# EternityJune25/ComoRAG

Hardware: AMD Instinct MI355X
Metric: top-k queries/sec (higher is better)
Workload: dtype bf16; 1 GPU; brute-force top-20 over 10000000 x 768 bf16 rows, batch 64, row-sharded over 1 GPU(s) (north_star target config); rows=10000000, dim=768, batch=64, k=20, query_batches_rotated=4, device=AMD Radeon Graphics (gfx950:sramecc+:xnack-), n_cu=256, repeats=1, exchange=none (1 shard)

## Files before the change

comorag_amd/csrc/api.hip:

```cpp
#include <hip/hip_runtime.h>

#include <algorithm>
#include <cmath>
#include <cstdarg>
#include <cstdio>
#include <cstdlib>
#include <cstring>
#include <chrono>
#include <atomic>
#include <climits>
#include <map>
#include <memory>
#include <mutex>
#include <shared_mutex>
#include <string>
#include <vector>

#include "../../include/comorag_hip.h"
#include "cmr_kernels.h"
#include "cmr_internal.h"
#include "index_state.h"
#include "search_plan.h"
#include "prefilter_host.h"

// ... 10 lines not shown
    g_err = buf;
    return code;
}
#define fail cmr_fail

int cmr_set_device(int device) {
    HIP_TRY(hipSetDevice(device));
    return CMR_OK;
}

namespace {

struct Option {
    const char* name;
    void (*store)(cmr_index*, long long);
    enum Kind { any, clamp, oneof, range, zero_or } kind;
    long long a, b, c;
    const char* reject;
    long long (*read)(const cmr_index*);
};
#define CMR_STR_(x) #x
#define CMR_STR(x) CMR_STR_(x)
#define OPT_FIELD(f) [](cmr_index* i, long long v) { i->f = (decltype(i->f))v; }
#define OPT_READ(expr) [](const cmr_index* i) -> long long { return expr; }
const Option kOptions[] = {
    {"scan_ring", OPT_FIELD(force_ring), Option::any, 0, 0, 0, nullptr, nullptr},
    {"scan_asm_ring", OPT_FIELD(force_asm), Option::any, 0, 0, 0, nullptr, nullptr},
    {"scan_grid", OPT_FIELD(force_grid), Option::any, 0, 0, 0, nullptr, nullptr},
    {"scan_no_sample", OPT_FIELD(no_sample), Option::any, 0, 0, 0, nullptr, nullptr},
    {"scan_no_wide", OPT_FIELD(no_wide), Option::any, 0, 0, 0, nullptr, nullptr},
    {"scan_no_tiny", OPT_FIELD(no_tiny), Option::any, 0, 0, 0, nullptr, nullptr},
    {"scan_no_small", OPT_FIELD(no_small), Option::any, 0, 0, 0, nullptr, nullptr},
    {"small_max_panels", OPT_FIELD(small_max_panels), Option::clamp, 32, 6144, 0, nullptr, nullptr},
    {"tiny_multi", OPT_FIELD(tiny_multi), Option::any, 0, 0, 0, nullptr, nullptr},
    {"zero_copy", OPT_FIELD(zero_copy), Option::any, 0, 0, 0, nullptr, nullptr},
    {"sample_single", OPT_FIELD(single_level), Option::any, 0, 0, 0, nullptr, nullptr},
    {"sample_single_max", OPT_FIELD(single_level_max), Option::clamp, 0, LLONG_MAX, 0, nullptr, nullptr},
    {"sample_tau_in_scan", OPT_FIELD(tau_in_scan), Option::any, 0, 0, 0, nullptr, nullptr},
    {"scan_fin", OPT_FIELD(scan_fin), Option::any, 0, 0, 0, nullptr, nullptr},
    {"sync_poll", OPT_FIELD(sync_poll), Option::any, 0, 0, 0, nullptr, nullptr},
    {"scan_fin_dense", OPT_FIELD(fin_dense), Option::clamp, 1, 1 << 16, 0, nullptr, nullptr},
    {"scan_fin_cap", OPT_FIELD(fin_cap), Option::oneof, 0, 128, 256, "scan_fin_cap must be 0, 128 or 256", nullptr},
    {"scan_fin_suppliers", OPT_FIELD(fin_suppliers), Option::clamp, 0, CMR_FIN_SLOTS / CMR_SCAN_WAVES, 0, nullptr, nullptr},
    {"scan_fin_spin", OPT_FIELD(fin_spin), Option::clamp, 0, 1000, 0, nullptr, nullptr},
    {"scan_fin_queries", OPT_FIELD(fin_max_q), Option::clamp, 1, CMR_FIN_MAX_QUERIES, 0, nullptr, nullptr},
    {"sample_div", OPT_FIELD(sample_div), Option::clamp, 2, LLONG_MAX, 0, nullptr, nullptr},
    {"sample_maxmul", OPT_FIELD(sample_maxmul), Option::clamp, 0, LLONG_MAX, 0, nullptr, nullptr},
    {"pipe_reserve_cus", OPT_FIELD(reserve_cus), Option::any, 0, 0, 0, nullptr, nullptr},
    {"pipe_slots", OPT_FIELD(pipe_slots), Option::any, 0, 0, 0, nullptr, nullptr},
    {"wide_mode", OPT_FIELD(wide_mode), Option::range, 0, 2, 0, "wide_mode must be 0 (default), 1 (register-resident kernel) or 2 (query-split grid)", nullptr},
    {"stream_nt", OPT_FIELD(stream_nt), Option::any, 0, 0, 0, nullptr, nullptr},
    {"pipe_dual_scan", OPT_FIELD(dual_scan), Option::any, 0, 0, 0, nullptr, nullptr},
    {"pipe_cu_mask", OPT_FIELD(cu_mask), Option::any, 0, 0, 0, nullptr, nullptr},
    {"exact_cand", OPT_FIELD(exact_cand), Option::range, 2, CMR_MAX_K, 0, "exact_cand must be in [2, " CMR_STR(CMR_MAX_K) "]", OPT_READ(i->exact_cand)},
    {"combine", [](cmr_index* i, long long v) { i->combine.store((int)v, std::memory_order_relaxed); }, Option::zero_or, 2, cmr_combine::kMaxWidth, 0,
     "combine must be 0 (off) or in [2, " CMR_STR(CMR_PPR_MAX_BATCH) "]", OPT_READ(i->combine.load(std::memory_order_relaxed))},
    {"combine_wait_us", [](cmr_index* i, long long v) { i->combine_wait_us.store(v, std::memory_order_relaxed); }, Option::clamp, 0, 10000000, 0, nullptr,
     OPT_READ(i->combine_wait_us.load(std::memory_order_relaxed))},
    {"combine_filtered", [](cmr_index* i, long long v) { i->combine_filtered.store((int)v, std::memory_order_relaxed); }, Option::range, 0, 1, 0,
     "combine_filtered must be 0 or 1", OPT_READ(i->combine_filtered.load(std::memory_order_relaxed))},
    {"prefilter", OPT_FIELD(prefilter), Option::range, -1, 2, 0, "prefilter must be -1 (auto), 0 (off), 1 (on) or 2 (on, the filter keeps every row)", OPT_READ(i->prefilter)},
    {"prefilter_rescore_wgs", OPT_FIELD(pf_rescore_wgs), Option::clamp, 0, 1024, 0, nullptr, nullptr},
    {"prefilter_tighten", OPT_FIELD(pf_tighten), Option::range, 0, 1, 0, "prefilter_tighten must be 0 or 1", OPT_READ(i->pf_tighten)},
    {"prefilter_pair_cap", OPT_FIELD(pf_pair_cap), Option::clamp, 0, 1 << 20, 0, nullptr, OPT_READ(i->pf_pair_cap)},
    {"prefilter_wave_cap", OPT_FIELD(pf_wave_cap), Option::clamp, 0, 1 << 20, 0, nullptr, OPT_READ(i->pf_wave_cap)},
    {"prefilter_sample", OPT_FIELD(pf_sample), Option::range, -1, 1, 0, "prefilter_sample must be -1 (auto), 0 (bf16 sampling) or 1 (int8 sample)", OPT_READ(i->pf_sample)},
    {"prefilter_sample_panels", OPT_FIELD(pf_sample_panels), Option::clamp, 0, INT_MAX, 0, nullptr, OPT_READ(i->pf_sample_panels)},
    {"prefilter_sample_run", OPT_FIELD(pf_sample_run), Option::clamp, 0, 1 << 16, 0, nullptr, OPT_READ(i->pf_sample_run)},
    {"prefilter_sample_wave_cap", OPT_FIELD(pf_sample_wave_cap), Option::clamp, 0, 1 << 20, 0, nullptr, OPT_READ(i->pf_sample_wave_cap)},
    {"prefilter_sample_level0", OPT_FIELD(pf_sample_level0), Option::clamp, 0, 128, 0, nullptr, OPT_READ(i->pf_sample_level0)},
    {"prefilter_sample_active", nullptr, Option::any, 0, 0, 0, nullptr, OPT_READ(i->prefilter_sample_active)},
    {"prefilter_sample_pairs", nullptr, Option::any, 0, 0, 0, nullptr, OPT_READ(q8_read_counter(i, Q8Counter::sample_pairs))},
    {"prefilter_sample_overflow", nullptr, Option::any, 0, 0, 0, nullptr, OPT_READ(q8_read_counter(i, Q8Counter::sample_overflow))},
    {"prefilter_active", nullptr, Option::any, 0, 0, 0, nullptr, OPT_READ(i->prefilter_active)},
    {"prefilter_rows", nullptr, Option::any, 0, 0, 0, nullptr, OPT_READ(i->q8c.q8 ? i->q8c.rows : 0)},
    {"prefilter_bytes", nullptr, Option::any, 0, 0, 0, nullptr, OPT_READ((long long)i->q8c.bytes(i->dpad))},
    {"prefilter_candidates", nullptr, Option::any, 0, 0, 0, nullptr, OPT_READ(q8_read_counter(i, Q8Counter::candidates))},
    {"prefilter_pairs", nullptr, Option::any, 0, 0, 0, nullptr, OPT_READ(q8_read_counter(i, Q8Counter::pairs))},
    {"prefilter_pair_overflow", nullptr, Option::any, 0, 0, 0, nullptr, OPT_READ(q8_read_counter(i, Q8Counter::pair_overflow))},
    {"prefilter_wave_overflow", nullptr, Option::any, 0, 0, 0, nullptr, OPT_READ(q8_read_counter(i, Q8Counter::wave_overflow))},
    {"last_route", nullptr, Option::any, 0, 0, 0, nullptr, OPT_READ(i->last_route.load(std::memory_order_relaxed))},
    {"pipe_dual_scan_active", nullptr, Option::any, 0, 0, 0, nullptr, OPT_READ(i->dual_active)},
    {"pipe_dual_scan_wide_active", nullptr, Option::any, 0, 0, 0, nullptr, OPT_READ(i->dual_wide_active)},
    {"pipe_cu_mask_active", nullptr, Option::any, 0, 0, 0, nullptr, OPT_READ(i->pipe.last_masked)},
    {"pipe_scan_cus", nullptr, Option::any, 0, 0, 0, nullptr, OPT_READ(i->pipe.last_masked ? i->pipe.scan_cus : i->n_cu)},
    {"combine_batches", nullptr, Option::any, 0, 0, 0, nullptr, OPT_READ(i->combiner.batches())},
    {"combine_queries", nullptr, Option::any, 0, 0, 0, nullptr, OPT_READ(i->combiner.queries())},
    {"combine_max_width", nullptr, Option::any, 0, 0, 0, nullptr, OPT_READ(i->combiner.max_width())},
};
#undef OPT_FIELD
#undef OPT_READ

const Option* find_option(const char* name) {
    for (const Option& o : kOptions) if (strcmp(o.name, name) == 0) return &o;
    return nullptr;
}

int set_option(cmr_index* idx, const char* name, long long v) {
    const Option* o = find_option(name ? name : "");
    if (!o || !o->store) return fail(CMR_ERR_INVALID, "unknown option '%s'", name ? name : "");
    const bool refused = o->kind == Option::oneof ? (v != o->a && v != o->b && v != o->c) : o->kind == Option::range ? (v < o->a || v > o->b) : o->kind == Option::zero_or ? (v != 0 && (v < o->a || v > o->b)) : false;
    if (refused) return fail(CMR_ERR_INVALID, "%s", o->reject);
    if (o->kind == Option::clamp) v = std::max(o->a, std::min(v, o->b));
    o->store(idx, v);
    return CMR_OK;
}
// ... 181 lines not shown
    {
        std::lock_guard<std::mutex> pg(idx->prof_mu);
        prof = idx->prof_on && (idx->prof_seq++ % (unsigned)idx->prof_every) == 0;
    }
    if (prof) {
        HIP_TRY(hipEventCreate(&pe.a));
        HIP_TRY(hipEventCreate(&pe.b));
        HIP_TRY(hipEventRecord(pe.a, sm));
    }
    const int* fin_state = nullptr;
    if (p.fin) {
        if (!ws->fin_ctl_armed) {
            HIP_TRY(ws->fin_ctl.ensure(p.bytes.fin_ctl));
            HIP_TRY(hipMemsetAsync(ws->fin_ctl.p, 0, p.bytes.fin_ctl, sm));
            ws->fin_ctl_armed = true;
        }
        HIP_TRY(ws->fin_pmax.ensure(p.bytes.fin_pmax));
        HIP_TRY(ws->fin_tau.ensure(p.bytes.fin_tau));
        HIP_TRY(ws->fin_mm.ensure(p.bytes.fin_mm));
        a.fin_mm = (u64*)ws->fin_mm.p;
        HIP_TRY(ws->fin_dense.ensure(p.bytes.fin_dense));
        a.fin = (int*)ws->fin_ctl.p; a.fin_pmax = (u64*)ws->fin_pmax.p; a.fin_tau = (u64*)ws->fin_tau.p; a.fin_dense = (u64*)ws->fin_dense.p;
        a.fin_first = p.fin_first; a.fin_wgs = p.fin_wgs; a.fin_mul = p.fin_mul; a.fin_dcap = p.fin_dcap; a.fin_spin = p.fin_spin;
        a.out_ids = ids_dev; a.out_scores = scores_dev; a.out_min = min_dev; a.out_max = max_dev; a.id_base = kernel_id_base(idx);
        fin_state = (const int*)ws->fin_ctl.p + CMR_FIN_STATE;
        if (ws->done_ptr && idx->single_block()) a.fin_done = ws->done_ptr;
    }
    if (p.prefilter) { if ((rc = q8_filter(idx, f, a, sm))) return rc; }
    else HIP_TRY(p.wide ? cmr_launch_scan_wide(g, a, sm) : p.fin ? cmr_launch_scan_fin(g, a, sm) : p.masked_each ? cmr_launch_scan_masked_each(g, a, sm) : p.masked ? cmr_launch_scan_masked(g, a, sm) : cmr_launch_scan_topk(g, a, sm));
    if (prof) {
        HIP_TRY(hipEventRecord(pe.b, sm));
        std::lock_guard<std::mutex> pg(idx->prof_mu);
        idx->prof_events.push_back(pe);
        idx->prof_bytes = p.prefilter ? prefilter_bytes(idx, p) : algorithmic_bytes(idx, nqp, k);
    }
    if (a.fin_done) {
        ws->lazy.due = true;
        ws->lazy.lists = (const u64*)ws->lists.p; ws->lazy.cnt = (const int*)ws->cnt.p; ws->lazy.W = p.W; ws->lazy.NQ = p.NQ; ws->lazy.cap = g.cap; ws->lazy.nqp = nqp; ws->lazy.k = k;
        ws->lazy.mm = (const float2*)ws->mm.p; ws->lazy.id_base = kernel_id_base(idx); ws->lazy.ids = ids_dev; ws->lazy.scores = scores_dev; ws->lazy.mn = min_dev; ws->lazy.mx = max_dev;
        ws->lazy.state = fin_state;
        ws->done_used = true;
        return CMR_OK;
    }
    if (sq != sm) {
        HIP_TRY(hipEventRecord(st.ev_scan, sm));
        HIP_TRY(hipStreamWaitEvent(sq, st.ev_scan, 0));
    }
    if (p.prefilter && (rc = q8_rescore(f, sq))) return rc;
    HIP_TRY(cmr_launch_merge_query((const u64*)ws->lists.p, (const int*)ws->cnt.p, p.W, p.NQ, g.cap, nqp, k, (const float2*)ws->mm.p,
                                   kernel_id_base(idx), ids_dev, scores_dev, min_dev, max_dev, nullptr, sq, G > 1, fin_state));
    return remap_ids_enqueue(idx, ids_dev, (long long)nqp * k, sq);
}

int plan_and_enqueue_pass(cmr_index* idx, Workspace* ws, const PassStreams& st, const PassSplit& ps, int k, int reserve_cus, const float* q_dev,
                          const float* min_score, int64_t* ids_dev, float* scores_dev, float* min_dev, float* max_dev, int prefilter = 0) {
    PassPlan plan;
    PassRequest rq = st.request(ps.nqp, k, ps.route, min_score != nullptr, reserve_cus);
    rq.prefilter = prefilter;
    int rc = plan_pass(idx, rq, &plan);
    if (rc) return rc;
    if (ps.q0 == 0)
        idx->last_route.store(route_code(plan, min_score != nullptr) | (ps.nqp < ps.nq ? CMR_ROUTE_MORE_PASSES : 0), std::memory_order_relaxed);
    return enqueue_pass(idx, ws, st, plan, q_dev + (size_t)ps.q0 * idx->dim, min_score, ids_dev + (size_t)ps.q0 * k, scores_dev + (size_t)ps.q0 * k,
                        min_dev ? min_dev + ps.q0 : nullptr, max_dev ? max_dev + ps.q0 : nullptr);
}

int search_enqueue(cmr_index* idx, Workspace* ws, const float* q_dev, int nq, int k, int64_t* ids_dev, float* scores_dev,
                   float* min_dev, float* max_dev, const float* min_score = nullptr) {
    if (k > CMR_MAX_K) {
        if (min_score) return fail(CMR_ERR_UNSUPPORTED, "threshold search supports k <= %d", CMR_MAX_K);
        return search_large_k_enqueue(idx, ws, q_dev, nq, k, ids_dev, scores_dev, min_dev, max_dev);
    }
    if (const int kind = small_path_kind(idx, nq, k, min_score != nullptr)) {
        const long long npanels = idx->npanels();
        idx->last_route.store(route_code(kind == 1 ? CMR_ROUTE_TINY : CMR_ROUTE_SMALL), std::memory_order_relaxed);
        { int rc_ = arm_flag(ws, ws->stream); if (rc_) return rc_; }
        HIP_TRY(ws->d_out.ensure(cmr_tiny_scratch_bytes(nq, (int)npanels, k, idx->tiny_multi, idx->small_max_panels)));
        if (!ws->arrive.p) {
            HIP_TRY(ws->arrive.ensure(sizeof(int)));
            HIP_TRY(hipMemsetAsync(ws->arrive.p, 0, sizeof(int), ws->stream));
        }
        HIP_TRY(cmr_launch_tiny_search(idx->dtype, idx->corpus, q_dev, nq, idx->dim, idx->dpad, idx->n, k, kernel_id_base(idx), ws->d_out.p,
                                       ids_dev, scores_dev, min_dev, max_dev, ws->flag_ptr, idx->tiny_multi ? (int*)ws->arrive.p : nullptr, idx->small_max_panels, ws->stream,
                                       (ws->done_ptr && idx->single_block()) ? ws->done_ptr : nullptr));
        if (ws->done_ptr && idx->single_block()) ws->done_used = true;
        return remap_ids_enqueue(idx, ids_dev, (long long)nq * k, ws->stream);
    }
    const PassStreams st = PassStreams::one(ws->stream);
    for (PassSplit ps(idx, nq); ps.next();) {
        int rc = plan_and_enqueue_pass(idx, ws, st, ps, k, 0, q_dev, min_score, ids_dev, scores_dev, min_dev, max_dev);
        if (rc) return rc;
    }
    return CMR_OK;
}

int search_masked_enqueue(cmr_index* idx, Workspace* ws, const float* q_dev, int nq, int k, const unsigned* allow_dev, int64_t* ids_dev,
                          float* scores_dev, float* min_dev, float* max_dev, long long mask_stride = 0) {
    const PassStreams st = PassStreams::one(ws->stream);
    const int per_pass = idx->narrow_width(nq);
    for (int q0 = 0; q0 < nq; q0 += per_pass) {
        const int nqp = std::min(per_pass, nq - q0);
        PassPlan plan;
        PassRequest rq = st.request(nqp, k, Route::narrow, false, 0);
        rq.masked = true;
        rq.masked_each = mask_stride > 0;
        int rc = plan_pass(idx, rq, &plan);
        if (rc) return rc;
        if (q0 == 0) idx->last_route.store(route_code(plan, false) | (nqp < nq ? CMR_ROUTE_MORE_PASSES : 0), std::memory_order_relaxed);
        rc = enqueue_pass(idx, ws, st, plan, q_dev + (size_t)q0 * idx->dim, nullptr, ids_dev + (size_t)q0 * k, scores_dev + (size_t)q0 * k,
                          min_dev ? min_dev + q0 : nullptr, max_dev ? max_dev + q0 : nullptr, allow_dev + (size_t)q0 * (size_t)mask_stride, mask_stride);
        if (rc) return rc;
    }
    return CMR_OK;
}

int create_pipe_streams(cmr_index* idx, Pipe& T, int mask, bool dual) {
    HIP_TRY(hipStreamCreateWithFlags(&T.st[Pipe::sq], hipStreamNonBlocking));
// ... 10 lines not shown
        uint32_t scan[8], rest[8];
        for (int w = 0; w < 8; ++w) {
            scan[w] = mask == 2 ? 0x00FFFFFFu : (w < 6 ? 0xFFFFFFFFu : 0u);
            rest[w] = ~scan[w];
        }
        HIP_TRY(hipExtStreamCreateWithCUMask(&T.st[Pipe::sm], 8, scan));
        if (dual) HIP_TRY(hipExtStreamCreateWithCUMask(&T.st[Pipe::sm2], 8, scan));
        HIP_TRY(hipExtStreamCreateWithCUMask(&T.st[Pipe::sp], 8, rest));
        T.scan_cus = idx->n_cu - 64;
        for (Pipe::Stream u : {Pipe::usp, Pipe::usm, Pipe::uwp, Pipe::uwm}) HIP_TRY(hipStreamCreateWithFlags(&T.st[u], hipStreamNonBlocking));
    } else {
        HIP_TRY(hipStreamCreateWithFlags(&T.st[Pipe::wp], hipStreamNonBlocking));
        HIP_TRY(hipStreamCreateWithFlags(&T.st[Pipe::wm], hipStreamNonBlocking));
        HIP_TRY(hipStreamCreateWithFlags(&T.st[Pipe::sp], hipStreamNonBlocking));
        HIP_TRY(hipStreamCreateWithFlags(&T.st[Pipe::sm], hipStreamNonBlocking));
        if (dual) HIP_TRY(hipStreamCreateWithFlags(&T.st[Pipe::sm2], hipStreamNonBlocking));
    }
    return CMR_OK;
}
int ensure_pipe(cmr_index* idx) {
    Pipe& P = idx->pipe;
    if (P.st[Pipe::sq]) return CMR_OK;
    int mask = idx->cu_mask < 0 ? (idx->n_cu == 256 ? 1 : 0) : (idx->n_cu == 256 ? idx->cu_mask : 0);
    hipEvent_t ev[CMR_PIPE_SLOTS][3] = {};
    Pipe T;
    auto undo = [&]() {
        T.destroy_streams();
        for (auto& slot : ev) for (hipEvent_t& e : slot) if (e) { (void)hipEventDestroy(e); e = nullptr; }
        T.scan_cus = T.wide_cus = 0;
    };
    int rc = create_pipe_streams(idx, T, mask, idx->dual_scan < 0 ? mask != 0 : idx->dual_scan != 0);
    if (rc && mask) {
        undo();
        mask = 0;
        rc = create_pipe_streams(idx, T, 0, idx->dual_scan > 0);
    }
    if (rc) { undo(); return rc; }
    auto make_events = [&]() -> int {
        for (auto& slot : ev) for (hipEvent_t& e : slot) HIP_TRY(hipEventCreateWithFlags(&e, hipEventDisableTiming));
        return CMR_OK;
    };
    rc = make_events();
    if (rc) { undo(); return rc; }
    for (int i = 0; i < Pipe::n_streams; ++i) if (i != Pipe::sq) P.st[i] = T.st[i];
    P.scan_cus = T.scan_cus; P.wide_cus = T.wide_cus;
    for (int i = 0; i < CMR_PIPE_SLOTS; ++i) {
        P.slot[i].pre_done = ev[i][0]; P.slot[i].main_done = ev[i][1]; P.slot[i].scan_done = ev[i][2];
        P.slot[i].ws.stream = P.st[Pipe::sm];
    }
    P.st[Pipe::sq] = T.st[Pipe::sq];
    return CMR_OK;
}

int search_pipelined_enqueue_locked(cmr_index* idx, const float* q_dev, int nq, int k, int64_t* ids_dev, float* scores_dev, float* min_dev,
                                    float* max_dev, hipEvent_t wait_event, hipEvent_t* done_event, const float* min_score, bool may_prefilter = false) {
    Pipe& P = idx->pipe;
    { int rc_ = ensure_pipe(idx); if (rc_) return rc_; }
    P.nslots = std::min(CMR_PIPE_SLOTS, std::max(2, idx->pipe_slots));
    if (k > CMR_MAX_K) return fail(CMR_ERR_UNSUPPORTED, "pipelined search supports k <= %d", CMR_MAX_K);
    const bool masked = P.scan_cus != 0 && (idx->cu_mask > 0 || idx->short_scan());
    const bool twins = P.scan_cus != 0 && !masked;
    P.last_masked = masked ? 1 : 0;
    hipStream_t const nsp = P.st[twins ? Pipe::usp : Pipe::sp], wsp = P.st[twins ? Pipe::uwp : Pipe::wp];
    PassSplit ps(idx, nq);
    if (wait_event) {
        HIP_TRY(hipStreamWaitEvent(nsp, wait_event, 0));
        if (ps.any_wide()) HIP_TRY(hipStreamWaitEvent(wsp, wait_event, 0));
    }
    int prefilter = prefilter_eligible(idx, min_score != nullptr, min_dev || max_dev, nq, may_prefilter);
    if (prefilter && !q8_ensure_companion(idx, nsp)) prefilter = 0;
    idx->prefilter_active = 0;
    idx->prefilter_sample_active = 0;
    PipeSlot* last = nullptr;
    while (ps.next()) {
        const bool wide = ps.wide_streams();
        PipeSlot* sl = &P.slot[P.next++ % (unsigned)P.nslots];
        hipStream_t sp = wide ? wsp : nsp;
        if (sl->used) {
            HIP_TRY(hipStreamWaitEvent(sp, sl->scan_done, 0));
        }
        const bool dual = !twins && P.st[wide ? Pipe::wm2 : Pipe::sm2] != nullptr && (idx->dual_scan > 0 || idx->short_scan());
        if (!wide) idx->dual_active = dual ? 1 : 0;
        else idx->dual_wide_active = dual ? 1 : 0;
        hipStream_t sm = P.st[twins ? (wide ? Pipe::uwm : Pipe::usm)
                                    : wide ? ((dual && (P.nwscan++ & 1)) ? Pipe::wm2 : Pipe::wm) : ((dual && (P.nscan++ & 1)) ? Pipe::sm2 : Pipe::sm)];
        const PassStreams st{sp, sm, P.st[Pipe::sq], sl->pre_done, sl->scan_done, sl->used ? sl->main_done : nullptr};
        int rc = plan_and_enqueue_pass(idx, &sl->ws, st, ps, k, (masked && !wide) ? idx->n_cu - P.scan_cus : (masked && wide) ? idx->n_cu - P.wide_cus : idx->reserve_cus,
                                       q_dev, min_score, ids_dev, scores_dev, min_dev, max_dev, wide ? 0 : prefilter);
        if (rc) return rc;
        HIP_TRY(hipEventRecord(sl->main_done, P.st[Pipe::sq]));
        sl->used = true;
        last = sl;
    }
    if (done_event) *done_event = last ? last->main_done : nullptr;
    return CMR_OK;
}
int search_pipelined_enqueue(cmr_index* idx, const float* q_dev, int nq, int k, int64_t* ids_dev, float* scores_dev, float* min_dev,
                             float* max_dev, hipEvent_t wait_event, hipEvent_t* done_event, const float* min_score = nullptr, bool may_prefilter = false) {
    std::lock_guard<std::mutex> pl(idx->pipe_mu);
    return search_pipelined_enqueue_locked(idx, q_dev, nq, k, ids_dev, scores_dev, min_dev, max_dev, wait_event, done_event, min_score, may_prefilter);
}

int scores_enqueue(cmr_index* idx, Workspace* ws, const float* q_dev, int nq, float* out_dev, long long ld) {
    hipStream_t s = ws->stream;
    CmrScanGeom g{};
    const int per_pass = idx->narrow_width(nq);
    const long long npanels = idx->npanels();
    { int rc_ = arm_flag(ws, s); if (rc_) return rc_; }
    for (int q0 = 0; q0 < nq; q0 += per_pass) {
        const int nqp = std::min(per_pass, nq - q0);
        int rc = make_geom(idx, nqp, 1, false, &g);
        if (rc) return rc;
        HIP_TRY(ws->qfrag.ensure((size_t)g.nqt * g.ks * 1024));
        HIP_TRY(cmr_launch_prep_queries(idx->dtype, q_dev + (size_t)q0 * idx->dim, nqp, idx->dim, idx->dpad, g.nqt, ws->qfrag.p,
                                        ws->flag_ptr, s));
        CmrScanArgs a{};
        a.corpus = idx->corpus; a.qfrag = ws->qfrag.p; a.nrows = idx->n; a.npanels = (int)npanels; a.k = 1;
        a.scores = out_dev + (size_t)q0 * ld; a.ld = ld; a.nq = nqp;
        HIP_TRY(cmr_launch_scan_scores(g, a, s));
    }
    return CMR_OK;
}

int check_query_flag(Workspace* ws) {
    int h = 0;
    HIP_TRY(hipMemcpyAsync(&h, ws->flag_ptr, sizeof(int), hipMemcpyDeviceToHost, ws->stream));
    HIP_TRY(hipStreamSynchronize(ws->stream));
    if (h) {
        HIP_TRY(hipMemsetAsync(ws->flag_ptr, 0, sizeof(int), ws->stream));
        return fail(CMR_ERR_NONFINITE, "query contains NaN/Inf or a value that rounds to Inf in the index dtype");
    }
    return CMR_OK;
}

int grow(cmr_index* idx, long long need_panels) {
    if (need_panels <= idx->cap_panels) return CMR_OK;
    long long new_cap = std::max(need_panels, idx->cap_panels * 2);
    new_cap = std::max<long long>(new_cap, 8);
    const size_t pb = idx->panel_bytes();
    HIP_TRY(hipDeviceSynchronize());
    void* nc = nullptr;
// ... 442 lines not shown
            return fail(CMR_ERR_UNSUPPORTED, "block %d reaches global id %lld: the packed candidate exchange carries 32-bit rows", b, (long long)(global_start[b] + len - 1));
    }
    if (n_blocks == 1) {
        idx->id_base = global_start[0];
        idx->blk_local.clear(); idx->blk_global.clear();
        return CMR_OK;
    }
    int rc = cmr_set_device(idx->device);
    if (rc) return rc;
    std::vector<long long> tab((size_t)2 * n_blocks);
    for (int b = 0; b < n_blocks; ++b) { tab[b] = local_start[b]; tab[n_blocks + b] = global_start[b]; }
    long long* d = nullptr;
    HIP_TRY(hipMalloc((void**)&d, tab.size() * 8));
    HIP_TRY(hipMemcpy(d, tab.data(), tab.size() * 8, hipMemcpyHostToDevice));
    if (idx->d_blk) idx->blk_retired.push_back(idx->d_blk);
    if (idx->blk_retired.size() >= 8) {
        HIP_TRY(hipDeviceSynchronize());
        for (void* p : idx->blk_retired) (void)hipFree(p);
        idx->blk_retired.clear();
    }
    idx->d_blk = d;
    idx->blk_local.assign(local_start, local_start + n_blocks);
    idx->blk_global.assign(global_start, global_start + n_blocks);
    idx->id_base = global_start[0];
    return CMR_OK;
}

int32_t cmr_index_set_option(cmr_index_t* idx, const char* name, int64_t value) {
    if (!idx || !name) return fail(CMR_ERR_INVALID, "NULL argument");
    std::unique_lock<std::shared_mutex> lk(idx->mu);
    return set_option(idx, name, value);
}

int32_t cmr_index_get_option(cmr_index_t* idx, const char* name, int64_t* value) {
    if (!idx || !name || !value) return fail(CMR_ERR_INVALID, "NULL argument");
    std::shared_lock<std::shared_mutex> lk(idx->mu);
    const Option* o = find_option(name);
    if (!o || !o->read) return fail(CMR_ERR_INVALID, "unknown readable option '%s'", name);
    *value = o->read(idx);
    return CMR_OK;
}

int32_t cmr_index_pipeline_stream(cmr_index_t* idx, int32_t which, void** stream) {
    if (!idx || !stream) return fail(CMR_ERR_INVALID, "NULL argument");
    if (which < 0 || which > 2) return fail(CMR_ERR_INVALID, "which must be 0 (pre), 1 (scan) or 2 (post)");
    int rc = cmr_set_device(idx->device);
    if (rc) return rc;
    std::lock_guard<std::mutex> pl(idx->pipe_mu);
    Pipe& P = idx->pipe;
    rc = ensure_pipe(idx);
    if (rc) return rc;
    const bool twins = P.scan_cus != 0 && !P.last_masked && P.next != 0;
    *stream = (void*)P.st[which == 0 ? (twins ? Pipe::usp : Pipe::sp) : which == 1 ? (twins ? Pipe::usm : Pipe::sm) : Pipe::sq];
    return CMR_OK;
}

int32_t cmr_index_query_status(cmr_index_t* idx, int32_t* nonfinite) {
    if (!idx || !nonfinite) return fail(CMR_ERR_INVALID, "NULL argument");
    *nonfinite = 0;
    std::shared_lock<std::shared_mutex> lk(idx->mu);
    int rc = cmr_set_device(idx->device);
    if (rc) return rc;
    std::vector<Workspace*> wss;
    {
        std::lock_guard<std::mutex> pl(idx->pipe_mu);
        for (int i = 0; i < CMR_PIPE_SLOTS; ++i) if (idx->pipe.slot[i].used) wss.push_back(&idx->pipe.slot[i].ws);
        if (idx->pipe.st[Pipe::sq]) {
            for (hipStream_t st : idx->pipe.st) if (st) HIP_TRY(hipStreamSynchronize(st));
        }
    }
    {
        std::lock_guard<std::mutex> g(idx->ws_mu);
        for (auto& kv : idx->stream_ws) wss.push_back(kv.second);
    }
    for (Workspace* ws : wss) {
        if (!ws->flag_ptr) continue;
        if (ws->stream || !ws->own_stream) HIP_TRY(hipStreamSynchronize(ws->stream));
        int h = 0;
        HIP_TRY(hipMemcpy(&h, ws->flag_ptr, sizeof(int), hipMemcpyDeviceToHost));
        if (h) {
            *nonfinite = 1;
            HIP_TRY(hipMemset(ws->flag_ptr, 0, sizeof(int)));
        }
    }
    return CMR_OK;
}

int32_t cmr_stream_wait_event(void* stream, void* event) {
    if (!event) return CMR_OK;
    HIP_TRY(hipStreamWaitEvent((hipStream_t)stream, (hipEvent_t)event, 0));
    return CMR_OK;
}

int32_t cmr_event_synchronize(void* event) {
    if (!event) return CMR_OK;
    HIP_TRY(hipEventSynchronize((hipEvent_t)event));
    return CMR_OK;
}

}

struct CmrPending {
    cmr_index* idx = nullptr;
    Workspace* ws = nullptr;
    bool locked = false;
    bool mapped = false;
// ... 895 lines not shown
```

comorag_amd/csrc/index_state.h:

```cpp
#pragma once
#include <hip/hip_runtime.h>

#include <algorithm>
#include <atomic>
#include <cstring>
#include <map>
#include <mutex>
#include <shared_mutex>
#include <vector>

#include "../../include/comorag_hip.h"
#include "cmr_kernels.h"
#include "cmr_internal.h"
#include "combine.h"

#define CMR_DT_F32 0
#define CMR_PANEL_ROWS 32
#define CMR_SCAN_WAVES 8
#define CMR_CORPUS_SLACK (128 * 1024)

namespace {

int elem_size(int dtype) { return dtype == CMR_F32 ? 4 : 2; }
int round_up(int x, int m) { return (x + m - 1) / m * m; }
// ... 32 lines not shown
    bool fin_ctl_armed = false;
    DevBuf d_q, d_ids, d_scores, d_min, d_max, d_cand, d_out;
    DevBuf d_mask;
    DevBuf d_lists;
    DevBuf d_pack;
    Q8Scratch q8;
    ExactScratch x;
    int* flag_ptr = nullptr;
    int* done_ptr = nullptr;
    bool done_used = false;
    struct LazyMerge {
        bool due = false;
        const u64* lists = nullptr; const int* cnt = nullptr; int W = 0, NQ = 0, cap = 0, nqp = 0, k = 0; const float2* mm = nullptr; long long id_base = 0;
        int64_t* ids = nullptr; float* scores = nullptr; float* mn = nullptr; float* mx = nullptr; const int* state = nullptr;
    } lazy;
    void* h_pin = nullptr;
    void* h_pin_dev = nullptr;
    size_t h_pin_cap = 0;
    hipError_t ensure_pin(size_t need) {
        if (need <= h_pin_cap) return hipSuccess;
        if (h_pin) { hipError_t e = hipHostFree(h_pin); if (e != hipSuccess) return e; h_pin = nullptr; h_pin_dev = nullptr; h_pin_cap = 0; }
        const size_t want = std::max(need, h_pin_cap * 2);
        hipError_t e = hipHostMalloc(&h_pin, want, hipHostMallocDefault);
        if (e != hipSuccess) return e;
        e = hipHostGetDevicePointer(&h_pin_dev, h_pin, 0);
        if (e != hipSuccess) { (void)hipHostFree(h_pin); h_pin = nullptr; return e; }
        h_pin_cap = want;
        return hipSuccess;
    }
    void release() {
        qfrag.release(); lists.release(); cnt.release(); mm.release(); flag.release(); tau.release();
        s_lists.release(); s_cnt.release(); s_mm.release(); arrive.release();
        fin_ctl.release(); fin_pmax.release(); fin_tau.release(); fin_dense.release(); fin_mm.release();
        d_q.release(); d_ids.release(); d_scores.release(); d_min.release(); d_max.release(); d_cand.release(); d_out.release();
        d_mask.release();
        d_lists.release();
        d_pack.release();
        q8.release();
        x.release();
        if (h_pin) (void)hipHostFree(h_pin);
        h_pin = nullptr; h_pin_dev = nullptr; h_pin_cap = 0;
        if (own_stream && stream) (void)hipStreamDestroy(stream);
    }
};

struct ProfEvent { hipEvent_t a, b; };

constexpr size_t kMappedAppendMax = 128 * 1024;
constexpr size_t kZeroCopyMax = 256 * 1024;

struct PipeSlot { Workspace ws; hipEvent_t pre_done = nullptr, scan_done = nullptr, main_done = nullptr; bool used = false; };
#define CMR_PIPE_SLOTS 4
struct Pipe {
    enum Stream { sp, sm, sm2, wp, wm, wm2, usp, usm, uwp, uwm, sq, n_streams };
    hipStream_t st[n_streams] = {};
    PipeSlot slot[CMR_PIPE_SLOTS]; unsigned next = 0; int nslots = 2; unsigned nscan = 0, nwscan = 0; int scan_cus = 0, wide_cus = 0; int last_masked = 0;
    void destroy_streams() { for (hipStream_t& s : st) if (s) { (void)hipStreamDestroy(s); s = nullptr; } }
};

}

struct cmr_index {
    int device = 0;
    int dim = 0, dpad = 0, dtype = 0;
    uint32_t flags = 0;
    int n_cu = 256;
    long long n = 0;
    long long cap_panels = 0;
    void* corpus = nullptr;
    float* shadow = nullptr;
    std::shared_mutex mu;
    std::mutex ws_mu;
    std::vector<Workspace*> free_ws;
    std::map<hipStream_t, Workspace*> stream_ws;
    DevBuf stage;
    void* h_pin = nullptr;
    void* h_pin_dev = nullptr;
    size_t h_pin_cap = 0;
    int* d_flag = nullptr;
    std::mutex prof_mu;
    bool prof_on = false;
    int prof_every = 1;
    unsigned prof_seq = 0;
    std::vector<ProfEvent> prof_events;
    double prof_bytes = 0.0;
    int force_ring = 0;
    int force_asm = -1;
    int force_grid = 0;
    int no_sample = 0;
    int no_wide = 0;
    int no_tiny = 0;
    long long single_level_max = 320000;
    int single_level = 1;
    int tiny_multi = 1;
    int small_max_panels = 6144;
    int no_small = 0;
    int zero_copy = 1;
    int dual_scan = -1;
    int cu_mask = -1;
    int stream_nt = -1;
    int wide_mode = 0;
    int tau_in_scan = 1;
    int sync_poll = 1;
    int scan_fin = 1;
    int fin_dense = 16384;
    int fin_cap = 0;
    int fin_suppliers = 0;
    int fin_spin = 0;
    int fin_max_q = 8;
    int dual_wide_active = 0;
    std::atomic<long long> last_route{0};
    int dual_active = 0;
    std::atomic<int> combine{0};
    std::atomic<long long> combine_wait_us{0};
    std::atomic<int> combine_filtered{0};
    cmr_combine::Combiner combiner;
    long long id_base = 0;
    std::vector<long long> blk_local, blk_global;
    long long* d_blk = nullptr;
    std::vector<void*> blk_retired;
    int sample_maxmul = 0;
    int sample_div = 32;
    int prefilter = -1;
    int pf_rescore_wgs = 0;
    int pf_tighten = 1;
    int pf_pair_cap = 16384;
    int pf_wave_cap = 0;
    int pf_sample = -1;
    int pf_sample_panels = 0;
    int pf_sample_run = 0;
    int pf_sample_wave_cap = 0;
    int pf_sample_level0 = 0;
    int prefilter_sample_active = 0;
    Q8Companion q8c;
    int prefilter_active = 0;
    Q8LastPass q8_last;
    int pipe_slots = 3;
    int reserve_cus = -1;
    std::mutex pipe_mu;
    Pipe pipe;
    float* d_stats = nullptr;
    int exact_cand = CMR_MAX_K;
    ExactScratch x_slot[CMR_PIPE_SLOTS];
    unsigned x_next = 0;

    size_t panel_bytes() const { return (size_t)CMR_PANEL_ROWS * dpad * elem_size(dtype); }
    long long npanels() const { return panels_of(n); }
    int ks() const { return dtype == CMR_F32 ? dpad / 8 : dpad / 16; }
    int narrow_max() const { return cmr_scan_max_nqt(dtype, dpad) >= 2 ? 64 : 32; }
    int narrow_width(int nq) const { return nq > 32 ? narrow_max() : 32; }
    double scan_us() const { return (double)npanels() * panel_bytes() / 6.0e6; }
    bool short_scan() const { return scan_us() < 1000.0; }
    bool single_block() const { return blk_local.size() <= 1; }
    bool small_operands_fit() const { return (size_t)ks() * 1024 <= 143 * 1024; }
};

namespace {

long long kernel_id_base(const cmr_index* idx) { return idx->single_block() ? idx->id_base : 0; }

Workspace* acquire_ws(cmr_index* idx, hipStream_t user_stream, bool dev_api) {
    std::lock_guard<std::mutex> g(idx->ws_mu);
    if (dev_api && user_stream) {
        auto it = idx->stream_ws.find(user_stream);
        if (it != idx->stream_ws.end()) return it->second;
        Workspace* w = new Workspace();
        w->stream = user_stream;
        idx->stream_ws[user_stream] = w;
        return w;
    }
    if (dev_api) {
        auto it = idx->stream_ws.find(nullptr);
        if (it != idx->stream_ws.end()) return it->second;
        Workspace* w = new Workspace();
        w->stream = nullptr;
        idx->stream_ws[nullptr] = w;
        return w;
    }
    if (!idx->free_ws.empty()) { Workspace* w = idx->free_ws.back(); idx->free_ws.pop_back(); return w; }
    Workspace* w = new Workspace();
    if (hipStreamCreateWithFlags(&w->stream, hipStreamNonBlocking) != hipSuccess) { delete w; return nullptr; }
    w->own_stream = true;
    return w;
}
void release_ws(cmr_index* idx, Workspace* w) {
    std::lock_guard<std::mutex> g(idx->ws_mu);
    idx->free_ws.push_back(w);
}

struct SyncCall {
    cmr_index* idx;
// ... 44 lines not shown
```

comorag_amd/csrc/search_plan.h:

```cpp
#pragma once
#include <numeric>

#include "index_state.h"

bool cmr_ring_audit_ok(int dtype, int nqt, int cap, int ring, int mode);
static const long long kMaxMergeLists = 4096;
constexpr bool kPrefilterSampleAuto = false;
static const long long kQ8SamplePanels = 8192;
static const int kQ8SampleRun = 16;
static const int kQ8SampleLevel0 = 64;

namespace {

int make_geom(const cmr_index* idx, int nq, int k, bool topk, CmrScanGeom* g) {
    const int max_nqt = cmr_scan_max_nqt(idx->dtype, idx->dpad);
    if (max_nqt == 0) return cmr_fail(CMR_ERR_UNSUPPORTED, "dim %d too large for the LDS-resident query tile (dtype %d)", idx->dim, idx->dtype);
    g->dtype = idx->dtype;
    g->dpad = idx->dpad;
    g->nqt = (nq > 32 && max_nqt >= 2) ? 2 : 1;
    g->cap = (topk && k > 32) ? 256 : 128;
    const int ks = idx->ks();
    g->ring = (ks % 16 == 0) ? 16 : 8;
    if (idx->force_ring == 8 || (idx->force_ring == 16 && ks % 16 == 0)) g->ring = idx->force_ring;
    const int mode = topk ? 0 : 1;
    g->asm_ring = cmr_ring_audit_ok(g->dtype, g->nqt, g->cap, g->ring, mode) ? 1 : 0;
    if (idx->force_asm == 0) g->asm_ring = 0;
    if (idx->force_asm == 1 && !cmr_ring_audit_ok(g->dtype, g->nqt, g->cap, g->ring, mode))
        return cmr_fail(CMR_ERR_UNSUPPORTED, "CMR_SCAN_ASM_RING=1 but variant (dtype %d nqt %d cap %d ring %d) failed the ISA audit", g->dtype, g->nqt, g->cap, g->ring);
    if (!cmr_scan_geom(g)) return cmr_fail(CMR_ERR_UNSUPPORTED, "scan geometry does not fit LDS (dpad %d nqt %d)", idx->dpad, g->nqt);
    const int bpc = g->lds <= 80 * 1024 ? 2 : 1;
    long long grid = (idx->npanels() + CMR_SCAN_WAVES - 1) / CMR_SCAN_WAVES;
    grid = std::min<long long>(grid, (long long)idx->n_cu * bpc);
    if (idx->force_grid > 0) grid = std::min<long long>(grid, idx->force_grid);
    g->grid = (int)std::max<long long>(grid, 1);
    return CMR_OK;
}

double algorithmic_bytes(const cmr_index* idx, int nq, int k) {
    return (double)idx->npanels() * CMR_PANEL_ROWS * idx->dpad * elem_size(idx->dtype) + (double)nq * idx->dim * 4 + (double)nq * k * 12;
}

int balanced_grid(long long npanels, int grid, int lists_per_wg) {
    int best = grid;
    double best_cost = -1.0;
    for (int g = grid; g >= std::max(1, grid - grid / 8); --g) {
        const long long W = (long long)g * lists_per_wg;
        const double cost = (double)((npanels + W - 1) / W * W) * (1.0 + 0.0005 * (grid - g));
        if (best_cost < 0 || cost < best_cost) { best_cost = cost; best = g; }
    }
    return best;
}


enum class Route { narrow, wide, quad };

struct PassRequest {
    int nqp = 0, k = 0;
    Route route = Route::narrow;
    bool has_min_score = false;
    bool single_stream = false;
    bool pipelined = false;
    int reserve_cus = 0;
    int prefilter = 0;
    bool masked = false;
    bool masked_each = false;
};

struct PassPlan {
    int nqp = 0, k = 0;
    bool wide = false;
    CmrScanGeom g{};
    bool fin = false;
    bool masked = false;
    bool masked_each = false;
    int prefilter = 0;
    int rescore_grid = 0;
    int pair_cap = 0;
    int wave_cap = 0;
    bool sample_q8 = false;
    int s_run = 0, s_stride = 0, s_nruns = 0, s_wave_cap = 0, s_pair_cap = 0;
    int G = 1;
    int n_levels = 0;
    struct Level { long long panels; int grid, Wl, clog, stride; } level[2] = {};
    bool single_level = false;
    bool tau_in_scan = false;
    int reserve_cus = 0;
    int lists_per_wg = CMR_SCAN_WAVES;
    int NQ = 0, W = 0, Ws = 0, tiles = 0, NQA = 0;
    int fin_first = 0, fin_wgs = 0, fin_mul = 1, fin_dcap = 0, fin_spin = 0;
    struct { size_t qfrag, lists, cnt, mm, s_lists, s_cnt, s_mm, tau, fin_ctl, fin_pmax, fin_tau, fin_mm, fin_dense, q8[Q8_NBUF]; } bytes = {};
};

int plan_pass(const cmr_index* idx, const PassRequest& rq, PassPlan* out) {
    PassPlan& p = *out;
    p = PassPlan{};
    const int nqp = rq.nqp, k = rq.k;
    const bool wide = rq.route == Route::wide, quad = rq.route == Route::quad;
    p.nqp = nqp; p.k = k; p.wide = wide;
    if (rq.masked && (wide || quad || rq.prefilter)) return cmr_fail(CMR_ERR_INVALID, "a filtered pass is a narrow pass without the pre-filter");
    if (rq.masked_each && !rq.masked) return cmr_fail(CMR_ERR_INVALID, "per-query allow words belong to a filtered pass");
    p.masked = rq.masked; p.masked_each = rq.masked_each;
    CmrScanGeom& g = p.g;
    const long long npanels = idx->npanels();
    int rc = make_geom(idx, quad ? std::min(nqp, idx->narrow_max()) : nqp, k, true, &g);
    if (rc) return rc;
    const int G = quad ? (nqp + g.nqt * 32 - 1) / (g.nqt * 32) : 1;
    p.G = G;
    g.stream_default_policy = idx->stream_nt < 0 ? (G > 1 ? 1 : 0) : (idx->stream_nt ? 0 : 1);
    const int lists_per_wg = wide ? 1 : CMR_SCAN_WAVES;
    p.lists_per_wg = lists_per_wg;
    bool fin = !rq.masked && idx->scan_fin && !idx->no_sample && !wide && G == 1 && !rq.has_min_score && rq.single_stream && g.nqt == 1 && nqp <= idx->fin_max_q &&
               k <= 64 && npanels >= 4096 && npanels >= (long long)idx->n_cu * 2 * CMR_SCAN_WAVES;
    if (fin) {
        if ((idx->fin_cap == 256 || idx->fin_cap == 128) && idx->fin_cap > g.cap) {
            CmrScanGeom g2 = g;
            g2.cap = idx->fin_cap;
            if (cmr_scan_geom(&g2) && g2.lds + CMR_FIN_LDS <= 160 * 1024) g = g2;
        }
        const bool ok = cmr_ring_audit_ok(g.dtype, 1, g.cap, g.ring, 2);
        if (idx->force_asm == 1 && !ok) fin = false;
        if (g.lds + CMR_FIN_LDS > 160 * 1024 || g.grid > 512) fin = false;
        else g.asm_ring = (ok && idx->force_asm != 0) ? 1 : 0;
    }
    p.fin = fin;
    const bool prefilter = rq.prefilter && !wide && G == 1 && !fin;
    const bool sample_q8 = prefilter && rq.prefilter == 1 && idx->pf_tighten && idx->pf_pair_cap > 0 && npanels >= 4096 &&
                           (idx->pf_sample < 0 ? kPrefilterSampleAuto : idx->pf_sample == 1);
    long long level_panels[2] = {0, 0};
    long long bf16_level1 = 0;
    int n_levels = 0;
    bool single_level = false;
    if (!idx->no_sample && npanels >= 256 && !rq.has_min_score && !fin) {
        const long long s0 = sample_q8 ? std::max<long long>(idx->pf_sample_level0 > 0 ? idx->pf_sample_level0 : kQ8SampleLevel0, k) : std::max<long long>(16, k);
        single_level = !wide && !prefilter && idx->single_level && k <= 32 && nqp <= 8 && npanels >= 4096 && (long long)nqp * npanels <= idx->single_level_max;
        level_panels[n_levels++] = single_level ? 128 : s0;
        if (npanels >= 4096 && !single_level) {
            const long long maxmul = idx->sample_maxmul > 0 ? idx->sample_maxmul : (wide ? 512 : prefilter ? kMaxMergeLists : 128);
            const long long b0 = std::max<long long>(16, k);
            long long s1 = std::min<long long>(std::max<long long>(npanels / idx->sample_div, 8 * b0), maxmul * b0);
            if (!wide) s1 = std::min<long long>(s1, kMaxMergeLists);
            if (s1 < npanels / 2) bf16_level1 = s1;
            if (sample_q8) {
                level_panels[n_levels++] = idx->pf_sample_panels > 0 ? std::min<long long>(idx->pf_sample_panels, npanels)
                                                                     : std::min<long long>(std::max<long long>(npanels / idx->sample_div, 8 * s0), kQ8SamplePanels);
            } else if (bf16_level1) level_panels[n_levels++] = bf16_level1;
        }
    }
    p.n_levels = n_levels;
    p.single_level = single_level;
    p.sample_q8 = sample_q8 && n_levels == 2;
    const long long max_sample = std::max(level_panels[0], p.sample_q8 ? 0 : level_panels[1]);
    int reserve_cus = rq.reserve_cus;
    if (reserve_cus < 0) {
        if (!max_sample) reserve_cus = 0;
        else if (wide) {
            reserve_cus = 32;
        } else if (prefilter && idx->scan_us() >= 1250.0) {
            reserve_cus = 32;
        } else {
            const long long rounds = (long long)((0.7 * idx->scan_us() - 200.0) / 200.0);
            const long long wgs = std::max<long long>(1, (max_sample + lists_per_wg - 1) / lists_per_wg) * G;
            reserve_cus = rounds >= 1 ? (int)std::min<long long>(64, std::max<long long>(8, (wgs + rounds - 1) / rounds)) : 64;
        }
    }
    p.reserve_cus = reserve_cus;
    auto sample_grid = [&](long long spn) -> int {
        if (!wide) return (int)((spn + lists_per_wg - 1) / lists_per_wg);
        const int cap_wgs = rq.pipelined && reserve_cus > 0 ? reserve_cus : idx->n_cu;
        return (int)std::min<long long>(spn, std::max<long long>(cap_wgs, (spn + 47) / 48));
    };
    const int Ws = max_sample ? std::max(sample_grid(level_panels[0]), n_levels > 1 && !p.sample_q8 ? sample_grid(level_panels[1]) : 0) * lists_per_wg : 0;
    int NQ, W, tiles;
    if (wide) {
        const int nqb = cmr_wide_queries(idx->dtype, idx->dpad);
        g.nqt = 1;
        g.grid = (int)std::max<long long>(1, std::min<long long>(npanels, idx->n_cu));
        if (reserve_cus > 0 && g.grid > idx->n_cu / 2) g.grid = std::max(g.grid - reserve_cus, idx->n_cu / 2);
        NQ = nqb; W = g.grid; tiles = nqb / 32;
    } else if (G > 1) {
        if (reserve_cus > 0 && g.grid > idx->n_cu / 2) g.grid = std::max(g.grid - reserve_cus, idx->n_cu / 2);
        int vg = g.grid / G;
        if (vg >= 8) vg &= ~7;
        g.grid = std::max(vg, 1);
        NQ = g.nqt * 32; W = g.grid * CMR_SCAN_WAVES; tiles = G * g.nqt;
    } else {
        if (reserve_cus > 0 && g.grid > idx->n_cu / 2) g.grid = std::max(g.grid - reserve_cus, idx->n_cu / 2);
        if (!idx->force_grid) g.grid = balanced_grid(npanels, g.grid, CMR_SCAN_WAVES);
        NQ = g.nqt * 32; W = g.grid * CMR_SCAN_WAVES; tiles = g.nqt;
    }
    if (prefilter) {
        p.prefilter = rq.prefilter;
        p.rescore_grid = idx->pf_rescore_wgs > 0 ? idx->pf_rescore_wgs : std::min(idx->n_cu, 1024);
        W = p.rescore_grid * cmr_q8_rescore_waves();
        p.pair_cap = (rq.prefilter == 1 && idx->pf_tighten) ? idx->pf_pair_cap : 0;
        p.bytes.q8[Q8_QPACK] = (size_t)2 * tiles * (idx->dpad / 32) * 1024;
        p.bytes.q8[Q8_QCONST] = (size_t)NQ * sizeof(float4);
        p.bytes.q8[Q8_CAND] = (size_t)idx->cap_panels * CMR_PANEL_ROWS * sizeof(unsigned);
        p.bytes.q8[Q8_NCAND] = sizeof(unsigned);
        const long long fw = (long long)g.grid * CMR_SCAN_WAVES;
        p.wave_cap = !p.pair_cap ? 0 : idx->pf_wave_cap > 0 ? idx->pf_wave_cap : (int)std::min<long long>(1 << 20, (((long long)NQ * p.pair_cap + fw - 1) / fw + 63) / 64 * 64);
        p.bytes.q8[Q8_WREC] = std::max<size_t>((size_t)fw * p.wave_cap * 16, 16);
        p.bytes.q8[Q8_WCNT] = (size_t)fw * sizeof(unsigned);
        p.bytes.q8[Q8_PAIR] = std::max<size_t>((size_t)NQ * p.pair_cap * 16, 16);
        p.bytes.q8[Q8_PAIRCNT] = (size_t)NQ * sizeof(unsigned);
        p.bytes.q8[Q8_KEEP] = (size_t)idx->cap_panels * sizeof(unsigned);
        p.bytes.q8[Q8_TAU] = (size_t)NQ * sizeof(float);
        if (p.sample_q8) {
            const long long s1 = level_panels[1];
            const long long run = std::min<long long>(idx->pf_sample_run > 0 ? idx->pf_sample_run : kQ8SampleRun, s1);
            long long nruns = (s1 + run - 1) / run, stride = npanels / nruns;
            if (stride < run) { stride = run; nruns = std::min(nruns, (npanels + run - 1) / run); }
            p.s_run = (int)run; p.s_stride = (int)stride; p.s_nruns = (int)nruns;
            p.s_wave_cap = idx->pf_sample_wave_cap > 0 ? idx->pf_sample_wave_cap : (int)std::min<long long>(1 << 20, (run * CMR_PANEL_ROWS * NQ / 16 + 63) / 64 * 64);
            p.s_pair_cap = p.pair_cap;
            const long long sw = (nruns + CMR_SCAN_WAVES - 1) / CMR_SCAN_WAVES * CMR_SCAN_WAVES;
            p.bytes.q8[Q8_SWREC] = (size_t)sw * p.s_wave_cap * 16;
            p.bytes.q8[Q8_SWCNT] = (size_t)sw * sizeof(unsigned);
            p.bytes.q8[Q8_SPAIR] = (size_t)NQ * p.s_pair_cap * 16;
            p.bytes.q8[Q8_SPAIRCNT] = (size_t)NQ * sizeof(unsigned);
        }
    }
    const int NQA = G * NQ;
    p.NQ = NQ; p.W = W; p.Ws = Ws; p.tiles = tiles; p.NQA = NQA;
    p.bytes.qfrag = (size_t)tiles * g.ks * 1024;
    p.bytes.lists = (size_t)W * NQA * g.cap * 8;
    p.bytes.cnt = (size_t)W * NQA * 4;
    p.bytes.mm = (size_t)W * NQA * 8;
    p.bytes.s_lists = (size_t)Ws * NQA * g.cap * 8;
    p.bytes.s_cnt = (size_t)Ws * NQA * 4;
    p.bytes.s_mm = (size_t)Ws * NQA * 8;
    p.bytes.tau = (size_t)2 * NQA * 8;
    for (int lv = 0; lv < n_levels; ++lv) {
        PassPlan::Level& L = p.level[lv];
        const long long spn = level_panels[lv];
        L.panels = spn;
        if (lv == 1 && p.sample_q8) {
            L.grid = (p.s_nruns + CMR_SCAN_WAVES - 1) / CMR_SCAN_WAVES; L.Wl = 0; L.clog = 0; L.stride = p.s_stride;
            continue;
        }
        L.grid = sample_grid(spn);
        L.Wl = L.grid * lists_per_wg;
        L.grid *= G;
        L.clog = spn >= 64 ? 3 : 0;
        const long long nchunks = (spn + (1 << L.clog) - 1) >> L.clog;
// ... 77 lines not shown
```

Measured before the change: 42710 queries/s.

## Hand off prefiltered scan passes to alternating full-CU streams in pipeline

Adds a 'filter handoff' mode for pipelined prefilter searches. When the prefilter scan is long (scan_us at least 1250 with reserve of 32 CUs, auto mode), the main scan/rescore work runs on one of two alternating streams created with an all-CU mask instead of the unmasked twin streams. Successive passes are chained through a tail event so ordering holds. The aim is to let consecutive batches' filter stages overlap across all CUs. The cost is extra streams and cross-stream dependencies, plus possible contention with the sampling work.

```diff
diff --git a/comorag_amd/csrc/api.hip b/comorag_amd/csrc/api.hip
--- a/comorag_amd/csrc/api.hip
+++ b/comorag_amd/csrc/api.hip
@@ -86,6 +86,8 @@
     {"stream_nt", OPT_FIELD(stream_nt), Option::any, 0, 0, 0, nullptr, nullptr},
     {"pipe_dual_scan", OPT_FIELD(dual_scan), Option::any, 0, 0, 0, nullptr, nullptr},
     {"pipe_cu_mask", OPT_FIELD(cu_mask), Option::any, 0, 0, 0, nullptr, nullptr},
+    {"pipe_filter_handoff", OPT_FIELD(filter_handoff), Option::range, -1, 1, 0, "pipe_filter_handoff must be -1 (auto), 0 (off) or 1 (on)", OPT_READ(i->filter_handoff)},
+    {"pipe_filter_handoff_active", nullptr, Option::any, 0, 0, 0, nullptr, OPT_READ(i->handoff_active)},
     {"exact_cand", OPT_FIELD(exact_cand), Option::range, 2, CMR_MAX_K, 0, "exact_cand must be in [2, " CMR_STR(CMR_MAX_K) "]", OPT_READ(i->exact_cand)},
     {"combine", [](cmr_index* i, long long v) { i->combine.store((int)v, std::memory_order_relaxed); }, Option::zero_or, 2, cmr_combine::kMaxWidth, 0,
      "combine must be 0 (off) or in [2, " CMR_STR(CMR_PPR_MAX_BATCH) "]", OPT_READ(i->combine.load(std::memory_order_relaxed))},
@@ -373,17 +375,20 @@
     return remap_ids_enqueue(idx, ids_dev, (long long)nqp * k, sq);
 }
 
-int plan_and_enqueue_pass(cmr_index* idx, Workspace* ws, const PassStreams& st, const PassSplit& ps, int k, int reserve_cus, const float* q_dev,
-                          const float* min_score, int64_t* ids_dev, float* scores_dev, float* min_dev, float* max_dev, int prefilter = 0) {
-    PassPlan plan;
-    PassRequest rq = st.request(ps.nqp, k, ps.route, min_score != nullptr, reserve_cus);
-    rq.prefilter = prefilter;
-    int rc = plan_pass(idx, rq, &plan);
-    if (rc) return rc;
+int enqueue_planned_pass(cmr_index* idx, Workspace* ws, const PassStreams& st, const PassPlan& plan, const PassSplit& ps, int k, const float* q_dev,
+                         const float* min_score, int64_t* ids_dev, float* scores_dev, float* min_dev, float* max_dev) {
     if (ps.q0 == 0)
         idx->last_route.store(route_code(plan, min_score != nullptr) | (ps.nqp < ps.nq ? CMR_ROUTE_MORE_PASSES : 0), std::memory_order_relaxed);
     return enqueue_pass(idx, ws, st, plan, q_dev + (size_t)ps.q0 * idx->dim, min_score, ids_dev + (size_t)ps.q0 * k, scores_dev + (size_t)ps.q0 * k,
                         min_dev ? min_dev + ps.q0 : nullptr, max_dev ? max_dev + ps.q0 : nullptr);
+}
+
+int plan_and_enqueue_pass(cmr_index* idx, Workspace* ws, const PassStreams& st, const PassSplit& ps, int k, int reserve_cus, const float* q_dev,
+                          const float* min_score, int64_t* ids_dev, float* scores_dev, float* min_dev, float* max_dev) {
+    PassPlan plan;
+    int rc = plan_pass(idx, st.request(ps.nqp, k, ps.route, min_score != nullptr, reserve_cus), &plan);
+    if (rc) return rc;
+    return enqueue_planned_pass(idx, ws, st, plan, ps, k, q_dev, min_score, ids_dev, scores_dev, min_dev, max_dev);
 }
 
 int search_enqueue(cmr_index* idx, Workspace* ws, const float* q_dev, int nq, int k, int64_t* ids_dev, float* scores_dev,
@@ -500,13 +505,32 @@
     return CMR_OK;
 }
 
+hipStream_t next_handoff_stream(Pipe& P) {
+    if (P.handoff_refused) return nullptr;
+    if (!P.st[Pipe::hf2]) {
+        uint32_t all[8];
+        for (uint32_t& w : all) w = 0xFFFFFFFFu;
+        hipStream_t a = nullptr, b = nullptr;
+        if (hipExtStreamCreateWithCUMask(&a, 8, all) != hipSuccess || hipExtStreamCreateWithCUMask(&b, 8, all) != hipSuccess) {
+            if (a) (void)hipStreamDestroy(a);
+            (void)hipGetLastError();
+            P.handoff_refused = true;
+            return nullptr;
+        }
+        P.st[Pipe::hf] = a; P.st[Pipe::hf2] = b;
+    }
+    return P.st[(P.nfilter++ & 1) ? Pipe::hf2 : Pipe::hf];
+}
+
 int search_pipelined_enqueue_locked(cmr_index* idx, const float* q_dev, int nq, int k, int64_t* ids_dev, float* scores_dev, float* min_dev,
                                     float* max_dev, hipEvent_t wait_event, hipEvent_t* done_event, const float* min_score, bool may_prefilter = false) {
     Pipe& P = idx->pipe;
     { int rc_ = ensure_pipe(idx); if (rc_) return rc_; }
     P.nslots = std::min(CMR_PIPE_SLOTS, std::max(2, idx->pipe_slots));
     if (k > CMR_MAX_K) return fail(CMR_ERR_UNSUPPORTED, "pipelined search supports k <= %d", CMR_MAX_K);
-    const bool masked = P.scan_cus != 0 && (idx->cu_mask > 0 || idx->short_scan());
+    int prefilter = prefilter_eligible(idx, min_score != nullptr, min_dev || max_dev, nq, may_prefilter);
+    const bool handoff_forced = prefilter && idx->filter_handoff > 0 && idx->cu_mask < 0;
+    const bool masked = P.scan_cus != 0 && (idx->cu_mask > 0 || idx->short_scan()) && !handoff_forced;
     const bool twins = P.scan_cus != 0 && !masked;
     P.last_masked = masked ? 1 : 0;
     hipStream_t const nsp = P.st[twins ? Pipe::usp : Pipe::sp], wsp = P.st[twins ? Pipe::uwp : Pipe::wp];
@@ -515,7 +539,6 @@
         HIP_TRY(hipStreamWaitEvent(nsp, wait_event, 0));
         if (ps.any_wide()) HIP_TRY(hipStreamWaitEvent(wsp, wait_event, 0));
     }
-    int prefilter = prefilter_eligible(idx, min_score != nullptr, min_dev || max_dev, nq, may_prefilter);
     if (prefilter && !q8_ensure_companion(idx, nsp)) prefilter = 0;
     idx->prefilter_active = 0;
     idx->prefilter_sample_active = 0;
@@ -532,9 +555,21 @@
         else idx->dual_wide_active = dual ? 1 : 0;
         hipStream_t sm = P.st[twins ? (wide ? Pipe::uwm : Pipe::usm)
                                     : wide ? ((dual && (P.nwscan++ & 1)) ? Pipe::wm2 : Pipe::wm) : ((dual && (P.nscan++ & 1)) ? Pipe::sm2 : Pipe::sm)];
-        const PassStreams st{sp, sm, P.st[Pipe::sq], sl->pre_done, sl->scan_done, sl->used ? sl->main_done : nullptr};
-        int rc = plan_and_enqueue_pass(idx, &sl->ws, st, ps, k, (masked && !wide) ? idx->n_cu - P.scan_cus : (masked && wide) ? idx->n_cu - P.wide_cus : idx->reserve_cus,
-                                       q_dev, min_score, ids_dev, scores_dev, min_dev, max_dev, wide ? 0 : prefilter);
+        PassStreams st{sp, sm, P.st[Pipe::sq], sl->pre_done, sl->scan_done, sl->used ? sl->main_done : nullptr};
+        PassPlan plan;
+        PassRequest rq = st.request(ps.nqp, k, ps.route, min_score != nullptr,
+                                    (masked && !wide) ? idx->n_cu - P.scan_cus : (masked && wide) ? idx->n_cu - P.wide_cus : idx->reserve_cus);
+        rq.prefilter = wide ? 0 : prefilter;
+        int rc = plan_pass(idx, rq, &plan);
+        if (rc) return rc;
+        if (twins && !wide) {
+            hipStream_t const hs = plan.handoff ? next_handoff_stream(P) : nullptr;
+            if (hs) st.sm = hs;
+            idx->handoff_active = hs ? 1 : 0;
+            if (P.tail_done && P.tail_stream != st.sm) HIP_TRY(hipStreamWaitEvent(st.sm, P.tail_done, 0));
+            P.tail_stream = st.sm; P.tail_done = sl->scan_done;
+        } else if (!wide) idx->handoff_active = 0;
+        rc = enqueue_planned_pass(idx, &sl->ws, st, plan, ps, k, q_dev, min_score, ids_dev, scores_dev, min_dev, max_dev);
         if (rc) return rc;
         HIP_TRY(hipEventRecord(sl->main_done, P.st[Pipe::sq]));
         sl->used = true;
@@ -1083,6 +1118,7 @@
     if (rc) return rc;
     const bool twins = P.scan_cus != 0 && !P.last_masked && P.next != 0;
     *stream = (void*)P.st[which == 0 ? (twins ? Pipe::usp : Pipe::sp) : which == 1 ? (twins ? Pipe::usm : Pipe::sm) : Pipe::sq];
+    if (which == 1 && twins && P.tail_stream) *stream = (void*)P.tail_stream;
     return CMR_OK;
 }
 
diff --git a/comorag_amd/csrc/index_state.h b/comorag_amd/csrc/index_state.h
--- a/comorag_amd/csrc/index_state.h
+++ b/comorag_amd/csrc/index_state.h
@@ -108,9 +108,11 @@
 struct PipeSlot { Workspace ws; hipEvent_t pre_done = nullptr, scan_done = nullptr, main_done = nullptr; bool used = false; };
 #define CMR_PIPE_SLOTS 4
 struct Pipe {
-    enum Stream { sp, sm, sm2, wp, wm, wm2, usp, usm, uwp, uwm, sq, n_streams };
+    enum Stream { sp, sm, sm2, wp, wm, wm2, usp, usm, uwp, uwm, hf, hf2, sq, n_streams };
     hipStream_t st[n_streams] = {};
     PipeSlot slot[CMR_PIPE_SLOTS]; unsigned next = 0; int nslots = 2; unsigned nscan = 0, nwscan = 0; int scan_cus = 0, wide_cus = 0; int last_masked = 0;
+    hipStream_t tail_stream = nullptr; hipEvent_t tail_done = nullptr;
+    unsigned nfilter = 0; bool handoff_refused = false;
     void destroy_streams() { for (hipStream_t& s : st) if (s) { (void)hipStreamDestroy(s); s = nullptr; } }
 };
 
@@ -193,6 +195,8 @@
     Q8LastPass q8_last;
     int pipe_slots = 3;
     int reserve_cus = -1;
+    int filter_handoff = -1;
+    int handoff_active = 0;
     std::mutex pipe_mu;
     Pipe pipe;
     float* d_stats = nullptr;
diff --git a/comorag_amd/csrc/search_plan.h b/comorag_amd/csrc/search_plan.h
--- a/comorag_amd/csrc/search_plan.h
+++ b/comorag_amd/csrc/search_plan.h
@@ -75,6 +75,7 @@
     bool masked_each = false;
     int prefilter = 0;
     int rescore_grid = 0;
+    bool handoff = false;
     int pair_cap = 0;
     int wave_cap = 0;
     bool sample_q8 = false;
@@ -151,12 +152,14 @@
     p.sample_q8 = sample_q8 && n_levels == 2;
     const long long max_sample = std::max(level_panels[0], p.sample_q8 ? 0 : level_panels[1]);
     int reserve_cus = rq.reserve_cus;
+    bool long_prefilter = false;
     if (reserve_cus < 0) {
         if (!max_sample) reserve_cus = 0;
         else if (wide) {
             reserve_cus = 32;
         } else if (prefilter && idx->scan_us() >= 1250.0) {
             reserve_cus = 32;
+            long_prefilter = true;
         } else {
             const long long rounds = (long long)((0.7 * idx->scan_us() - 200.0) / 200.0);
             const long long wgs = std::max<long long>(1, (max_sample + lists_per_wg - 1) / lists_per_wg) * G;
@@ -190,6 +193,7 @@
     }
     if (prefilter) {
         p.prefilter = rq.prefilter;
+        p.handoff = rq.pipelined && (idx->filter_handoff < 0 ? long_prefilter : idx->filter_handoff != 0);
         p.rescore_grid = idx->pf_rescore_wgs > 0 ? idx->pf_rescore_wgs : std::min(idx->n_cu, 1024);
         W = p.rescore_grid * cmr_q8_rescore_waves();
         p.pair_cap = (rq.prefilter == 1 && idx->pf_tighten) ? idx->pf_pair_cap : 0;
```

Result: faster. 43140 queries/s (median of 6 runs) (+1.0%).
